# aspuru-guzik-group/waveflow

Hardware: AMD Instinct MI355X
Metric: flow log-prob evals/sec (higher is better)
Workload: dtype f32

## Files before the change

### waveflow_amd/build.py

```python
import os
import subprocess
import sys
from concurrent.futures import ThreadPoolExecutor

HERE = os.path.dirname(os.path.abspath(__file__))
CSRC = os.path.join(HERE, "csrc")
LIB = os.path.join(HERE, "libwaveflow_hip.so")
OBJ = os.path.join(CSRC, "_obj")

SOURCES = ["wf_tables.cpp", "wf_runtime.cpp", "wf_model_build.cpp", "wf_model_images.cpp", "wf_dispatch.cpp", "wf_train.cpp", "wf_kernels_scalar.hip", "wf_scalar_inst_d2.hip", "wf_scalar_inst_d3.hip", "wf_scalar_inst_d4.hip", "wf_scalar_inst_d56.hip",
           "wf_scalar_inst_d78.hip", "wf_scalar_inst_n64.hip", "wf_scalar_inst_n64_d56.hip",
           "wf_scalar_inst_n64_d78.hip", "wf_kernels_mfma.hip", "wf_mfma_inst_d2.hip", "wf_mfma_inst_d2t2.hip", "wf_mfma_inst_d34.hip",
           "wf_mfma_inst_d567.hip", "wf_mfma_inst_d8.hip", "wf_mfma_inst_k2.hip", "wf_kernels_rqs.hip", "wf_kernels_grad.hip", "wf_kernels_wave.hip", "wf_kernels_etile.hip",
           "wf_kernels_etile_bwd.hip", "wf_etile_bwd_k2.hip", "wf_kernels_etile_sample.hip", "wf_kernels_etile_dir.hip", "wf_kernels_spline.hip"]
FLAGS = ["--offload-arch=gfx950", "-O3", "-std=c++17", "-fPIC", "-ffp-contract=off", "-Wall", "-Wno-unused-function"]
FLAGS += ["-mllvm", "-amdgpu-prealloc-sgpr-spill-vgprs"]
FLAGS += os.environ.get("WF_CXXFLAGS", "").split()
MFMA_FLAGS = ["-fno-slp-vectorize", "-Xclang", "-target-feature", "-Xclang", "-packed-fp32-ops"]
EXTRA_FLAGS = {"wf_etile_bwd_k2.hip": ["-mllvm", "-amdgpu-sched-strategy=max-ilp"]}


def _hipcc():
    for c in (os.environ.get("HIPCC"), "/opt/rocm/bin/hipcc", "hipcc"):
        if c and (os.path.isabs(c) and os.path.exists(c) or not os.path.isabs(c)):
            return c
    return "hipcc"


def _deps(obj):
    try:
        text = open(obj + ".d").read()
    except OSError:
        return None
    words = text.replace("\\\n", " ").split()
    if len(words) < 2 or not words[0].endswith(":"):
        return None
    return words[1:]


def _stale(obj):
    deps = _deps(obj)
    try:
        t = os.path.getmtime(obj)
        return deps is None or any(os.path.getmtime(d) > t for d in deps)
    except OSError:
        return True


STAMP = os.path.join(HERE, "libwaveflow_hip.flags")


def _flags_text():
    return " ".join(FLAGS) + " | " + " ".join(MFMA_FLAGS) + " | " + " ".join(f"{k}: {' '.join(v)}" for k, v in sorted(EXTRA_FLAGS.items()))


def _library_current():
    try:
        if open(STAMP).read() != _flags_text():
            return False
        t = os.path.getmtime(LIB)
    except OSError:
        return False
    deps = [os.path.join(CSRC, f) for f in os.listdir(CSRC) if f.endswith((".hip", ".cpp", ".h"))]
    deps.append(os.path.join(HERE, "..", "include", "waveflow_hip.h"))
    return all(os.path.getmtime(d) <= t for d in deps if os.path.exists(d))


def build(force=False, verbose=False):
    if not force and _library_current():
        return LIB
    os.makedirs(OBJ, exist_ok=True)
    try:
        force = force or open(STAMP).read() != _flags_text()
    except OSError:
        force = True
    srcs = [s for s in SOURCES if os.path.exists(os.path.join(CSRC, s))]
    jobs = []
    for s in srcs:
        o = os.path.join(OBJ, s + ".o")
        if force or _stale(o):
            cmd = [_hipcc()] + FLAGS + (MFMA_FLAGS if ("mfma" in s or "etile" in s) else []) + EXTRA_FLAGS.get(s, []) + (["-x", "hip"] if s.endswith(".cpp") else [])
            cmd += ["-MD", "-MF", o + ".d", "-c", os.path.join(CSRC, s), "-o", o]
            jobs.append(cmd)

    def run(cmd):
        if verbose:
            print(" ".join(cmd), flush=True)
        r = subprocess.run(cmd, capture_output=True, text=True)
        if r.returncode != 0:
            raise RuntimeError("hipcc failed:\n" + " ".join(cmd) + "\n" + r.stdout + r.stderr)
        return r

    if jobs:
        with ThreadPoolExecutor(max_workers=min(os.cpu_count() or 4, 16, len(jobs))) as ex:
            list(ex.map(run, jobs))
    objs = [os.path.join(OBJ, s + ".o") for s in srcs]
    if jobs or force or not os.path.exists(LIB) or any(os.path.getmtime(LIB) < os.path.getmtime(o) for o in objs):
        tmp = LIB + ".tmp"
        run([_hipcc(), "--offload-arch=gfx950", "-shared", "-fPIC", "-o", tmp] + objs)
        if os.environ.get("WF_SKIP_ISA_GUARD") != "1":
            import importlib.util
            spec = importlib.util.spec_from_file_location("wf_isa_guard", os.path.join(HERE, "isa_guard.py"))
            isa_guard = importlib.util.module_from_spec(spec)
            spec.loader.exec_module(isa_guard)
            try:
                isa_guard.check(tmp)
            except Exception:
                os.remove(tmp)
                raise
        os.replace(tmp, LIB)
    with open(STAMP, "w") as f:
        f.write(_flags_text())
    return LIB


if __name__ == "__main__":
    print(build(force="--force" in sys.argv, verbose=True))
```

### waveflow_amd/csrc/wf_kernels_scalar.hip

```cpp
#include "wf_scalar_impl.h"

namespace wf {

namespace scalar {
WF_SCALAR_SHAPE(extern, 2, 32) WF_SCALAR_SHAPE(extern, 3, 32) WF_SCALAR_SHAPE(extern, 4, 32) WF_SCALAR_SHAPE(extern, 5, 32)
WF_SCALAR_SHAPE(extern, 6, 32) WF_SCALAR_SHAPE(extern, 7, 32) WF_SCALAR_SHAPE(extern, 8, 32)
WF_SCALAR_SHAPE(extern, 2, 64) WF_SCALAR_SHAPE(extern, 3, 64) WF_SCALAR_SHAPE(extern, 4, 64) WF_SCALAR_SHAPE(extern, 5, 64)
WF_SCALAR_SHAPE(extern, 6, 64) WF_SCALAR_SHAPE(extern, 7, 64) WF_SCALAR_SHAPE(extern, 8, 64)
}

namespace {
using namespace scalar;

constexpr int kSumBlock = 256;
constexpr int kSumMaxBlocks = 1024;

__device__ __forceinline__ void block_reduce2(double& a, double& b, double* sm) {
    sm[threadIdx.x] = a;
    sm[kSumBlock + threadIdx.x] = b;
    __syncthreads();
    for (int s = kSumBlock / 2; s > 0; s >>= 1) {
        if ((int)threadIdx.x < s) {
            sm[threadIdx.x] += sm[threadIdx.x + s];
            sm[kSumBlock + threadIdx.x] += sm[kSumBlock + threadIdx.x + s];
        }
        __syncthreads();
    }
    a = sm[0];
    b = sm[kSumBlock];
}

__device__ __forceinline__ void ring_push(double s, double q, double n, double* __restrict__ ring, int ring_len, unsigned long long* __restrict__ counter) {
    const unsigned long long c = *counter;
    double* slot = ring + (c % (unsigned long long)ring_len) * 3;
    slot[0] = s; slot[1] = q; slot[2] = n;
    *counter = c + 1;
}

__global__ __launch_bounds__(kSumBlock) void k_sums_stage1(const float* __restrict__ v, int64_t B, double* __restrict__ partial,
                                                           double* __restrict__ final, double* __restrict__ ring, int ring_len,
                                                           unsigned long long* __restrict__ counter) {
    __shared__ double sm[2 * kSumBlock];
    double s = 0.0, q = 0.0;
    for (int64_t i = (int64_t)blockIdx.x * kSumBlock + threadIdx.x; i < B; i += (int64_t)gridDim.x * kSumBlock) {
        const double x = (double)v[i];
        s += x;
        q += x * x;
    }
    block_reduce2(s, q, sm);
    if (threadIdx.x == 0) {
        if (final) {
            final[0] = s;
            final[1] = q;
            final[2] = (double)B;
            if (ring) ring_push(s, q, (double)B, ring, ring_len, counter);
        } else {
            partial[2 * blockIdx.x] = s;
            partial[2 * blockIdx.x + 1] = q;
        }
    }
}

__global__ __launch_bounds__(kSumBlock) void k_sums_stage2(const double* __restrict__ partial, int n_blocks, int64_t B, double* __restrict__ out,
                                                           double* __restrict__ ring, int ring_len, unsigned long long* __restrict__ counter) {
    __shared__ double sm[2 * kSumBlock];
    double s = 0.0, q = 0.0;
    for (int i = threadIdx.x; i < n_blocks; i += kSumBlock) {
        s += partial[2 * i];
        q += partial[2 * i + 1];
    }
    block_reduce2(s, q, sm);
    if (threadIdx.x == 0) {
        out[0] = s;
        out[1] = q;
        out[2] = (double)B;
        if (ring) ring_push(s, q, (double)B, ring, ring_len, counter);
    }
}

int sums_blocks(int64_t B) {
    int64_t n = (B + kSumBlock - 1) / kSumBlock;
    if (n < 1) n = 1;
    if (n > kSumMaxBlocks) n = kSumMaxBlocks;
    return (int)n;
}

int finish_launch() {
    hipError_t e = hipGetLastError();
    if (e != hipSuccess) {
        set_hip_error((int)e);
        return WF_ERR_HIP;
    }
    return WF_OK;
}

}

#define WF_DISPATCH_D(D_, NBP_, CALL)                                         \
    if ((NBP_) == 32) {                                                          \
        switch (D_) {                                                            \
            case 2: CALL(2, 32); break;                                          \
            case 3: CALL(3, 32); break;                                          \
            case 4: CALL(4, 32); break;                                          \
            case 5: CALL(5, 32); break;                                          \
            case 6: CALL(6, 32); break;                                          \
            case 7: CALL(7, 32); break;                                          \
            case 8: CALL(8, 32); break;                                          \
            default: return WF_ERR_UNSUPPORTED;                                  \
        }                                                                        \
    } else if ((NBP_) == 64) {                                                   \
        switch (D_) {                                                            \
            case 2: CALL(2, 64); break;                                          \
            case 3: CALL(3, 64); break;                                          \
            case 4: CALL(4, 64); break;                                          \
            case 5: CALL(5, 64); break;                                          \
            case 6: CALL(6, 64); break;                                          \
            case 7: CALL(7, 64); break;                                          \
            case 8: CALL(8, 64); break;                                          \
            default: return WF_ERR_UNSUPPORTED;                                  \
        }                                                                        \
    } else {                                                                     \
        return WF_ERR_UNSUPPORTED;                                               \
    }

int launch_scalar(const ModelDev& md, const ModelDev* md_dev, int mode, const float* x, int64_t B, float* out, float* u, int32_t* idx,
                  void* stream) {
    hipStream_t s = (hipStream_t)stream;
#define CALL(DD, NN) run_eval<DD, NN>(md_dev, mode, x, B, out, u, idx, s)
    WF_DISPATCH_D(md.D, md.nbp, CALL)
#undef CALL
    return finish_launch();
}

int launch_scalar_layer(const ModelDev& md, const ModelDev* md_dev, int layer, const float* u_in, int64_t B, float* y, float* logdet,
                        int32_t* idx, void* stream) {
    hipStream_t s = (hipStream_t)stream;
#define CALL(DD, NN) run_layer<DD, NN>(md_dev, layer, u_in, B, y, logdet, idx, s)
    WF_DISPATCH_D(md.D, md.nbp, CALL)
#undef CALL
    return finish_launch();
}

int launch_scalar_inverse(const ModelDev& md, const ModelDev* md_dev, const float* u, int64_t B, float* x, int exact, void* stream) {
    hipStream_t s = (hipStream_t)stream;
#define CALL(DD, NN) run_inverse<DD, NN>(md_dev, u, B, x, exact, s)
    WF_DISPATCH_D(md.D, md.nbp, CALL)
#undef CALL
    return finish_launch();
}

int launch_scalar_sample(const ModelDev& md, const ModelDev* md_dev, unsigned long long seed, int64_t B, float* x, float* latent, int exact,
                         void* stream) {
    hipStream_t s = (hipStream_t)stream;
#define CALL(DD, NN) run_sample<DD, NN>(md_dev, seed, B, x, latent, exact, s)
    WF_DISPATCH_D(md.D, md.nbp, CALL)
#undef CALL
    return finish_launch();
}

__global__ void k_sort_rows(const float* __restrict__ x, int64_t B, int D, float* __restrict__ xs, int32_t* __restrict__ inv) {
    const int64_t b = (int64_t)blockIdx.x * blockDim.x + threadIdx.x;
    if (b >= B) return;
    float r[WF_MAX_DIM];
    for (int d = 0; d < D; ++d) r[d] = x[b * D + d];
    int n = 0;
    for (int pass = 0; pass < D; ++pass)
        for (int i = pass & 1; i + 1 < D; i += 2)
            if (r[i] > r[i + 1]) {
                const float t = r[i]; r[i] = r[i + 1]; r[i + 1] = t;
                ++n;
            }
    if (xs)
        for (int d = 0; d < D; ++d) xs[b * D + d] = r[d];
    if (inv) inv[b] = n;
}
__global__ void k_apply_sign(float* __restrict__ v, const int32_t* __restrict__ inv, int64_t B) {
    const int64_t b = (int64_t)blockIdx.x * blockDim.x + threadIdx.x;
    if (b < B && (inv[b] & 1)) v[b] = -v[b];
}

int launch_sort_rows(const float* x, int64_t B, int D, float* xs, int32_t* inv, void* stream) {
    if (B <= 0) return WF_OK;
    hipLaunchKernelGGL(k_sort_rows, dim3((unsigned)((B + 255) / 256)), dim3(256), 0, (hipStream_t)stream, x, B, D, xs, inv);
    return finish_launch();
}
int launch_apply_sign(float* v, const int32_t* inv, int64_t B, void* stream) {
    if (B <= 0) return WF_OK;
    hipLaunchKernelGGL(k_apply_sign, dim3((unsigned)((B + 255) / 256)), dim3(256), 0, (hipStream_t)stream, v, inv, B);
    return finish_launch();
}

int64_t block_sums_ws_bytes(int64_t) { return (int64_t)kSumMaxBlocks * 2 * sizeof(double); }

int launch_block_sums(const float* v, int64_t B, double* out, void* ws, int64_t, void* stream, double* ring, int ring_len,
                      unsigned long long* counter) {
    hipStream_t s = (hipStream_t)stream;
    const int nb = sums_blocks(B);
    double* partial = (double*)ws;
    if (nb == 1) {
        hipLaunchKernelGGL(k_sums_stage1, dim3(1), dim3(kSumBlock), 0, s, v, B, partial, out, ring, ring_len, counter);
        return finish_launch();
    }
    hipLaunchKernelGGL(k_sums_stage1, dim3(nb), dim3(kSumBlock), 0, s, v, B, partial, (double*)nullptr, (double*)nullptr, 0,
                       (unsigned long long*)nullptr);
    hipLaunchKernelGGL(k_sums_stage2, dim3(1), dim3(kSumBlock), 0, s, (const double*)partial, nb, B, out, ring, ring_len, counter);
    return finish_launch();
}

}
```

### waveflow_amd/csrc/wf_mfma_impl.h

```cpp
#pragma once
#include <hip/hip_runtime.h>

#include <cstdlib>

#include "wf_internal.h"

#define WF_PIN() __builtin_amdgcn_sched_barrier(0)

namespace wf {
namespace mfma {

using f32x16 = __attribute__((ext_vector_type(16))) float;
using f32x4 = __attribute__((ext_vector_type(4))) float;
using i32x2 = __attribute__((ext_vector_type(2))) int;
using f32x2 = __attribute__((ext_vector_type(2))) float;
using f16x8 = __attribute__((ext_vector_type(8))) _Float16;

__device__ __forceinline__ float act_tanh(float xs) {
    return __builtin_fmaf(-2.0f, __builtin_amdgcn_rcpf(__builtin_amdgcn_exp2f(xs) + 1.0f), 1.0f);
}
__device__ __forceinline__ float act_sigmoid(float xs) {
    return __builtin_amdgcn_rcpf(1.0f + __builtin_amdgcn_exp2f(xs));
}
__device__ __forceinline__ float fast_log(float x) {
    return __builtin_amdgcn_logf(x) * 0.6931471805599453f;
}

__device__ __forceinline__ float xhalf_sum(float v) {
    const unsigned u = __float_as_uint(v);
    const auto s = __builtin_amdgcn_permlane32_swap(u, u, false, false);
    return __uint_as_float(s[0]) + __uint_as_float(s[1]);
}

__device__ __forceinline__ f32x4 load4(const float* p) { return *reinterpret_cast<const f32x4*>(p); }
__device__ __forceinline__ float uniform_f(float v) {
    float r;
    asm("v_readfirstlane_b32 %0, %1" : "=s"(r) : "v"(v));
    return r;
}
__device__ __forceinline__ float xhalf_max(float v) {
    const unsigned u = __float_as_uint(v);
    const auto s = __builtin_amdgcn_permlane32_swap(u, u, false, false);
    return fmaxf(__uint_as_float(s[0]), __uint_as_float(s[1]));
}

__device__ __forceinline__ f32x16 load16(const float* p) {
    const f32x4* q = reinterpret_cast<const f32x4*>(p);
    const f32x4 a = q[0], b = q[1], c = q[2], d = q[3];
    return f32x16{a[0], a[1], a[2], a[3], b[0], b[1], b[2], b[3], c[0], c[1], c[2], c[3], d[0], d[1], d[2], d[3]};
}

struct Lerp {
    int il, ir, xl, xr;
    float t;
};

__device__ __forceinline__ int wrap_clamp(int i, int n) {
    if (i < 0) i += n;
    return min(max(i, 0), n - 1);
}

__device__ __forceinline__ float div_by_n(float xl, float n, float rn, int exact_div) {
    if (exact_div) return xl / n;
    const float q = xl * rn;
    const float r = __builtin_fmaf(-q, n, xl);
    return __builtin_fmaf(r, rn, q);
}

__device__ __forceinline__ Lerp make_lerp(float x, int n_mesh, float rn, int exact_div) {
    Lerp L;
    const int n_points = n_mesh - 1;
    const float xs = x * (float)n_points;
    const float fl = floorf(xs);
    L.xl = (int)fl;
    L.xr = (int)ceilf(xs);
    L.il = wrap_clamp(L.xl, n_mesh);
    L.ir = wrap_clamp(L.xr, n_mesh);
    const float dx = x - div_by_n(fl, (float)n_points, rn, exact_div);
    L.t = L.il == L.ir ? 0.0f : dx * (float)n_points;
    return L;
}

__device__ __forceinline__ bool any_far(const Lerp& Lp);
__device__ __forceinline__ f32x2 comp_lerp(const f32x4* __restrict__ comp2, const Lerp& Lp) {
    const f32x4 c = comp2[Lp.il];
    float b0 = c[2], b1 = c[3];
    if (any_far(Lp)) {
        const f32x4 r = comp2[Lp.ir];
        const bool far = Lp.ir != Lp.il && Lp.ir != Lp.il + 1;
        b0 = far ? r[0] : b0;
        b1 = far ? r[1] : b1;
    }
    return f32x2{__builtin_fmaf(b0 - c[0], Lp.t, c[0]), __builtin_fmaf(b1 - c[1], Lp.t, c[1])};
}

struct Frag {
    f16x8 hi[2], lo[2];
};
using u32x4 = __attribute__((ext_vector_type(4))) unsigned;
using f16x2 = __attribute__((ext_vector_type(2))) _Float16;
__device__ __forceinline__ void split8(const float (&r)[8], f16x8& hi, f16x8& lo) {
    u32x4 H, L;
    asm volatile(
        "s_nop 0\n\t"
        "v_cvt_pk_f16_f32 %0, %8, %9\n\tv_cvt_pk_f16_f32 %1, %10, %11\n\tv_cvt_pk_f16_f32 %2, %12, %13\n\tv_cvt_pk_f16_f32 %3, %14, %15\n\t"
        "v_fma_mixhi_f16 %4, %0, -1.0, %9 op_sel:[1,0,0] op_sel_hi:[1,0,0]\n\t"
        "v_fma_mixhi_f16 %5, %1, -1.0, %11 op_sel:[1,0,0] op_sel_hi:[1,0,0]\n\t"
        "v_fma_mixhi_f16 %6, %2, -1.0, %13 op_sel:[1,0,0] op_sel_hi:[1,0,0]\n\t"
        "v_fma_mixhi_f16 %7, %3, -1.0, %15 op_sel:[1,0,0] op_sel_hi:[1,0,0]\n\t"
        "v_fma_mixlo_f16 %4, %0, -1.0, %8 op_sel_hi:[1,0,0]\n\t"
        "v_fma_mixlo_f16 %5, %1, -1.0, %10 op_sel_hi:[1,0,0]\n\t"
        "v_fma_mixlo_f16 %6, %2, -1.0, %12 op_sel_hi:[1,0,0]\n\t"
        "v_fma_mixlo_f16 %7, %3, -1.0, %14 op_sel_hi:[1,0,0]\n\t"
        "s_nop 1"
        : "=&v"(H[0]), "=&v"(H[1]), "=&v"(H[2]), "=&v"(H[3]), "=&v"(L[0]), "=&v"(L[1]), "=&v"(L[2]), "=&v"(L[3])
        : "v"(r[0]), "v"(r[1]), "v"(r[2]), "v"(r[3]), "v"(r[4]), "v"(r[5]), "v"(r[6]), "v"(r[7]));
    hi = __builtin_bit_cast(f16x8, H);
    lo = __builtin_bit_cast(f16x8, L);
}
template <int T>
__device__ __forceinline__ void mfma_step(const _Float16* Wh, const _Float16* Wl, int kt, int s, const Frag (&in)[T][2], f32x16 (&acc)[T], int lane) {
    const f16x8 ah = *reinterpret_cast<const f16x8*>(Wh + ((kt * 2 + s) * 64 + lane) * 8);
    const f16x8 al = *reinterpret_cast<const f16x8*>(Wl + ((kt * 2 + s) * 64 + lane) * 8);
#pragma unroll
    for (int t = 0; t < T; ++t) acc[t] = __builtin_amdgcn_mfma_f32_32x32x16_f16(al, in[t][kt].hi[s], acc[t], 0, 0, 0);
#pragma unroll
    for (int t = 0; t < T; ++t) acc[t] = __builtin_amdgcn_mfma_f32_32x32x16_f16(ah, in[t][kt].lo[s], acc[t], 0, 0, 0);
#pragma unroll
    for (int t = 0; t < T; ++t) acc[t] = __builtin_amdgcn_mfma_f32_32x32x16_f16(ah, in[t][kt].hi[s], acc[t], 0, 0, 0);
}
template <int T>
__device__ __forceinline__ void dense64_block(const _Float16* Wh, const _Float16* Wl, const Frag (&in)[T][2], f32x16 (&acc)[T], int lane) {
#pragma unroll
    for (int kt = 0; kt < 2; ++kt)
#pragma unroll
        for (int s = 0; s < 2; ++s) mfma_step<T>(Wh, Wl, kt, s, in, acc, lane);
}
template <int T>
__device__ __forceinline__ void act8(const f32x16 (&x)[T], int s, Frag (&f)[T][2], int ob) {
#pragma unroll
    for (int t = 0; t < T; ++t) {
        float r[8];
#pragma unroll
        for (int j = 0; j < 8; ++j) r[j] = __builtin_amdgcn_rcpf(__builtin_amdgcn_exp2f(x[t][8 * s + j]) + 1.0f);
        split8(r, f[t][ob].hi[s], f[t][ob].lo[s]);
    }
}

template <int D, int NBK>
struct NetOff {
    static constexpr int S0 = (D + 1) / 2;
    static constexpr int W0 = 0;
    static constexpr int b0 = W0 + 2 * S0 * 64;
    static constexpr int W1h = b0 + 64;
    static constexpr int W1l = W1h + 2048;
    static constexpr int b1 = W1l + 2048;
    static constexpr int W2h = b1 + 64;
    static constexpr int W2l = W2h + (D - 1) * NBK * 1024;
// ... 90 lines not shown
    WF_PIN();
    mfma_step<T>(W2h, W2l, 1, 0, h2, o, lane);
    mfma_step<T>(W2h, W2l, 1, 1, h2, o, lane);
}

__device__ __forceinline__ int med3i(int x, int lo, int hi) {
    int r;
    asm("v_med3_i32 %0, %1, %2, %3" : "=v"(r) : "v"(x), "v"(lo), "v"(hi));
    return r;
}
template <int NBK, int NO, bool FAR>
__device__ __forceinline__ void fetch_block(f32x16 (&A)[NO], f32x16 (&Bv)[NO], const float* __restrict__ tab, const Lerp& Lp, int h, const float* bnd, int kb) {
    const char* tb = reinterpret_cast<const char*>(tab);
    constexpr unsigned kRec = 32u * NO, kMesh = 8u * NBK * kRec;
    const bool far = FAR && Lp.ir != Lp.il && Lp.ir != Lp.il + 1;
#pragma unroll
    for (int q = 0; q < 4; ++q) {
        const i32x2 lh = *reinterpret_cast<const i32x2*>(bnd + (kb * 2 + h) * 16 + q * 2);
        const unsigned off = (unsigned)med3i(Lp.il, lh[0], lh[1]) * kMesh + (unsigned)(8 * kb + 2 * q + h) * kRec;
        unsigned offb = off + 16u;
        if (FAR) {
            const unsigned offr = (unsigned)med3i(Lp.ir, lh[0], lh[1]) * kMesh + (unsigned)(8 * kb + 2 * q + h) * kRec;
            offb = far ? offr : offb;
        }
#pragma unroll
        for (int o = 0; o < NO; ++o) {
            const f32x4 a = load4(reinterpret_cast<const float*>(tb + off + o * 32)), b = load4(reinterpret_cast<const float*>(tb + offb + o * 32));
#pragma unroll
            for (int e = 0; e < 4; ++e) { A[o][q * 4 + e] = a[e]; Bv[o][q * 4 + e] = b[e]; }
        }
    }
}
template <int NO>
__device__ __forceinline__ void block_dot(const f32x16& v, const f32x16 (&A)[NO], const f32x16 (&Bv)[NO], float t, float (&part)[NO]) {
    float sa[NO][2], sb[NO][2];
#pragma unroll
    for (int o = 0; o < NO; ++o) sa[o][0] = sa[o][1] = sb[o][0] = sb[o][1] = 0.0f;
#pragma unroll
    for (int r = 0; r < 16; r += 2)
#pragma unroll
        for (int o = 0; o < NO; ++o) {
            sa[o][0] = __builtin_fmaf(v[r], A[o][r], sa[o][0]);
            sb[o][0] = __builtin_fmaf(v[r], Bv[o][r], sb[o][0]);
            sa[o][1] = __builtin_fmaf(v[r + 1], A[o][r + 1], sa[o][1]);
            sb[o][1] = __builtin_fmaf(v[r + 1], Bv[o][r + 1], sb[o][1]);
        }
#pragma unroll
    for (int o = 0; o < NO; ++o) {
        const float Aa = sa[o][0] + sa[o][1], Bb = sb[o][0] + sb[o][1];
        part[o] += __builtin_fmaf(Bb - Aa, t, Aa);
    }
}
template <int NBK, int NO, bool FAR>
__device__ __forceinline__ void rows_lerp_dot(const f32x16 (&v)[NBK], const float* __restrict__ tab, const Lerp& Lp, int h, const float* bnd, float (&out)[NO],
                                              const float* __restrict__ rsum = nullptr, float* rl = nullptr, float* rr = nullptr) {
    auto row_sums = [&]() {
        if (rsum) {
            static_assert(NO <= 2, "row sums: orders 0 and 1");
            const f32x4 c = load4(rsum + (size_t)Lp.il * 4);
            f32x4 r = c;
            bool far = false;
            if (FAR) {
                far = Lp.ir != Lp.il && Lp.ir != Lp.il + 1;
                r = load4(rsum + (size_t)Lp.ir * 4);
            }
#pragma unroll
            for (int o = 0; o < NO; ++o) {
                rl[o] = c[o];
                rr[o] = far ? r[o] : c[2 + o];
            }
        }
    };
    float part[NO];
#pragma unroll
    for (int o = 0; o < NO; ++o) part[o] = 0.0f;
    if (NBK > 1) row_sums();
#pragma unroll
    for (int kb = 0; kb < NBK; ++kb) {
        f32x16 A[NO], Bv[NO];
        if (kb > 0) __builtin_amdgcn_sched_barrier(0);
        fetch_block<NBK, NO, FAR>(A, Bv, tab, Lp, h, bnd, kb);
        if (NBK == 1) row_sums();
        block_dot<NO>(v[kb], A, Bv, Lp.t, part);
    }
#pragma unroll
    for (int o = 0; o < NO; ++o) out[o] = xhalf_sum(part[o]);
}
__device__ __forceinline__ bool any_far(const Lerp& Lp) { return __builtin_amdgcn_ballot_w64(Lp.ir != Lp.il && Lp.ir != Lp.il + 1) != 0; }

template <int NBK>
__device__ __forceinline__ float rows_dot(const f32x16 (&v)[NBK], const float* __restrict__ tab, const Lerp& Lp, int h, const float* bnd) {
    float out[1];
    if (!any_far(Lp)) rows_lerp_dot<NBK, 1, false>(v, tab, Lp, h, bnd, out);
    else rows_lerp_dot<NBK, 1, true>(v, tab, Lp, h, bnd, out);
    return out[0];
}

template <int NBK>
__device__ __forceinline__ void ispline_eval(const f32x16 (&v)[NBK], const float* __restrict__ tab, const float* __restrict__ rsum, const Lerp& Lp, int h,
                                             const float* bnd, float rS, float rs, float& y, float& logdy) {
    float num[2], rl[2], rr[2];
    if (!any_far(Lp)) rows_lerp_dot<NBK, 2, false>(v, tab, Lp, h, bnd, num, rsum, rl, rr);
    else rows_lerp_dot<NBK, 2, true>(v, tab, Lp, h, bnd, num, rsum, rl, rr);
    const float ynum = __builtin_fmaf(rs, __builtin_fmaf(rr[0] - rl[0], Lp.t, rl[0]), num[0]);
    const float dnum = __builtin_fmaf(rs, __builtin_fmaf(rr[1] - rl[1], Lp.t, rl[1]), num[1]);
    y = ynum * rS;
    logdy = fast_log(__builtin_fmaf(dnum, rS, 1e-7f));
}

template <int NBK>
__device__ __forceinline__ void sigmoid_block(f32x16 (&o)[NBK], const float* fk_lds , int h, float& S1, float& Sf,
                                              bool gate = false, float g = 1.0f, const float* z_lds = nullptr) {
    float s1 = 0.0f, sf = 0.0f;
#pragma unroll
    for (int kb = 0; kb < NBK; ++kb) {
        const f32x16 fk = load16(fk_lds + (kb * 2 + h) * 16);
        f32x16 zz = fk;
        if (gate) zz = load16(z_lds + (kb * 2 + h) * 16);
#pragma unroll
        for (int r = 0; r < 16; ++r) {
            float v = act_sigmoid(o[kb][r]);
            if (gate) v = __builtin_fmaf(g, v, zz[r]);
            o[kb][r] = v;
            s1 += v;
            sf = __builtin_fmaf(v, fk[r], sf);
        }
    }
    S1 = xhalf_sum(s1);
    Sf = xhalf_sum(sf);
}

template <int kThreads>
__device__ __forceinline__ void stage_floats(const float* __restrict__ src, float* dst, int n_floats) {
    const f32x4* s4 = reinterpret_cast<const f32x4*>(src);
    f32x4* d4 = reinterpret_cast<f32x4*>(dst);
    const int n4 = n_floats >> 2;
    for (int base = threadIdx.x; base < n4; base += kThreads * 8) {
        f32x4 v[8];
#pragma unroll
        for (int u = 0; u < 8; ++u) {
            const int i = base + u * kThreads;
            if (i < n4) v[u] = s4[i];
        }
#pragma unroll
        for (int u = 0; u < 8; ++u) {
            const int i = base + u * kThreads;
            if (i < n4) d4[i] = v[u];
        }
    }
}

template <int D, int NBK, int kWaves, int T, bool IDX, bool SPEC>
__global__ __launch_bounds__(kWaves * 64) void k_mfma(const MfmaDev mm, int mode_in, const float* __restrict__ xg, int64_t B,
                                                      float* __restrict__ out, float* __restrict__ u_out, int32_t* __restrict__ idx_out) {
    const int mode = mode_in & 3;
    const bool presort = (mode_in & 4) != 0;
    extern __shared__ __attribute__((aligned(16))) float lds[];
    constexpr int kThreads = kWaves * 64;
    const int box_kind = SPEC ? (int)WF_BOX_MEAN : mm.box_kind, layer_kind = SPEC ? (int)WF_LAYER_IMADE : mm.layer_kind;
    const int prior_kind = SPEC ? (int)WF_PRIOR_WAVEFLOW : mm.prior_kind, staged = (SPEC && D == 2) ? 0 : mm.staged, exact_div = SPEC ? 0 : mm.exact_div;
    __shared__ int next_slot;
    if (threadIdx.x == 0) next_slot = 0;
    stage_floats<kThreads>(mm.image + mm.const_img_off, lds, mm.const_floats);
    if (!staged) stage_floats<kThreads>(mm.image, lds + mm.const_floats, mm.net_floats * mm.n_nets);
    __syncthreads();

    const int lane = threadIdx.x & 63, wave = threadIdx.x >> 6;
    const int j = lane & 31, h = lane >> 5;
    const float* fkI = lds;
    const float* fkP = lds + 32 * NBK;
    const float* ob2b = lds + 64 * NBK;
    const float* bndI = ob2b + NBK * NBK * 1024;
    const float* bndP = bndI + 32 * NBK;
    const float* cbP = bndP + 32 * NBK;
    float* slots = lds + mm.const_floats;
    const int64_t n_tiles = (B + 31) >> 5;
    constexpr int kTilesPerChunk = kWaves * T;
    const int64_t n_chunks = (n_tiles + kTilesPerChunk - 1) / kTilesPerChunk;
    const int idx_stride = (mm.n_layers + 1) * D * 2;
    const float L = mm.box_L, tol = 1e-7f;
    const float rn_mesh = 1.0f / (float)(mm.n_mesh - 1);
    const float box_space0 = uniform_f(2 * L + tol), box_nlog0 = uniform_f(0.0f - fast_log(2 * L + tol));
    int f16_bad = 0;
    if (mm.f16_ovf)
        for (int n = 0; n < mm.n_nets; ++n) f16_bad |= mm.f16_ovf[n];
    const int64_t my_chunks = n_chunks > (int64_t)blockIdx.x ? (n_chunks - blockIdx.x + gridDim.x - 1) / gridDim.x : 0;
    const int my_slots = (int)(my_chunks * kWaves);
    auto tile_ids = [&](int64_t chunk, int wpos, int64_t (&w)[T], bool (&valid)[T], int32_t* (&idx)[T]) __attribute__((always_inline)) {
#pragma unroll
        for (int t = 0; t < T; ++t) {
            const int64_t tile = (chunk * kWaves + wpos) * T + t;
            w[t] = tile * 32 + j;
            valid[t] = w[t] < B;
            idx[t] = (IDX && idx_out && valid[t] && h == 0) ? idx_out + w[t] * idx_stride : nullptr;
        }
    };
    auto load_box = [&](const int64_t (&w)[T], const bool (&valid)[T], float (&cur)[T][D], float (&logdet)[T]) __attribute__((always_inline)) {
        float nxt[T][D];
#pragma unroll
        for (int t = 0; t < T; ++t) {
            const int64_t wl = valid[t] ? w[t] : B - 1;
#pragma unroll
            for (int d = 0; d < D; ++d) cur[t][d] = xg[wl * D + d];
            if (presort) {
#pragma unroll
                for (int r = 0; r < D; ++r)
#pragma unroll
                    for (int i = r & 1; i + 1 < D; i += 2) {
                        const float a = cur[t][i], b = cur[t][i + 1];
                        const bool sw = a > b;
                        cur[t][i] = sw ? b : a;
                        cur[t][i + 1] = sw ? a : b;
                    }
            }
        }
#pragma unroll
        for (int t = 0; t < T; ++t) {
            float ld = 0.0f;
            if (box_kind == WF_BOX_MEAN) {
                float s = 0.0f;
#pragma unroll
                for (int d = 0; d < D; ++d) s = s + cur[t][d];
                const float mean = s / (float)D;
                const float l = mean - cur[t][0];
                const float wd = cur[t][D - 1] - cur[t][0];
                float space_left = 2 * L;
#pragma unroll
                for (int i = 0; i < D - 1; ++i) {
                    const float diff = cur[t][i + 1] - cur[t][i];
                    nxt[t][i] = diff / (i == 0 ? box_space0 : space_left + tol);
                    ld = i == 0 ? box_nlog0 : ld - fast_log(space_left + tol);
                    space_left = space_left - diff;
                }
                nxt[t][D - 1] = (mean + L - l) / (2 * L - wd + tol);
                ld = ld - fast_log(2 * L - wd + tol);
#pragma unroll
                for (int d = 0; d < D; ++d) cur[t][d] = nxt[t][d];
            } else if (box_kind == WF_BOX_FIRST) {
                nxt[t][0] = (cur[t][0] + L) / (2 * L);
                float ls = 0.0f;
#pragma unroll
                for (int i = 1; i < D; ++i) nxt[t][i] = (cur[t][i] - cur[t][i - 1]) / (L - cur[t][i - 1] + tol);
#pragma unroll
                for (int i = 0; i < D - 1; ++i) ls = ls + fast_log(L - cur[t][i] + tol);
                ld = -fast_log(2 * L) - ls;
#pragma unroll
                for (int d = 0; d < D; ++d) cur[t][d] = nxt[t][d];
            }
            logdet[t] = ld;
        }

    };
    auto flow_layer = [&](int l, const float* net, float (&cur)[T][D], float (&logdet)[T], int32_t* (&idx)[T]) __attribute__((always_inline)) {
        float nxt[T][D];
        {
            Frag h2[T][2];
            f32x16 pend[T];
            hidden_layers<D, NBK, T>(net, cur, lane, h2, pend);
            if (layer_kind == WF_LAYER_IMADE) {
#pragma unroll
                for (int t = 0; t < T; ++t) {
                    const Lerp Lp = make_lerp(cur[t][0], mm.n_mesh, rn_mesh, exact_div);
                    if (IDX && idx[t]) { idx[t][(l * D) * 2] = Lp.xl; idx[t][(l * D) * 2 + 1] = Lp.xr; }
                    const f32x2 c0 = comp_lerp(mm.comp2 + (size_t)l * mm.n_mesh, Lp);
                    nxt[t][0] = c0[0];
                    logdet[t] = logdet[t] + fast_log(c0[1] + 1e-7f);
                }
                const bool gate_i = !SPEC && mm.i_gate != 0;
                float gl[T];
#pragma unroll
                for (int t = 0; t < T; ++t) gl[t] = 1.0f;
#pragma unroll (D)
                for (int d = 1; d < D; ++d) {
                    if (D > 4) __builtin_amdgcn_sched_barrier(0);
                    if (gate_i) {
#pragma unroll
                        for (int t = 0; t < T; ++t) gl[t] = gl[t] * (cur[t][d - 1] * cur[t][d - 1] * cur[t][d - 1]);
                    }
                    f32x16 v[T][NBK];
#pragma unroll
                    for (int kb = 0; kb < NBK; ++kb) {
                        f32x16 o[T];
                        if (d == 1 && kb == 0) out_block_first<D, NBK, T>(net, h2, pend, lane, o);
                        else out_block<D, NBK, T>(net, h2, d, kb, lane, o);
#pragma unroll
                        for (int t = 0; t < T; ++t) v[t][kb] = o[t];
                    }
#pragma unroll
                    for (int t = 0; t < T; ++t) {
                        float S1, Sf;
                        sigmoid_block<NBK>(v[t], fkI, h, S1, Sf, gate_i, gl[t], net + NetOff<D, NBK>::z + d * NBK * 32);
                        const float rs = mm.i_reg * S1;
                        const float rS = __builtin_amdgcn_rcpf(__builtin_fmaf(rs, mm.F_I, Sf));
                        const Lerp Lp = make_lerp(cur[t][d], mm.n_mesh, rn_mesh, exact_div);
                        if (IDX && idx[t]) { idx[t][(l * D + d) * 2] = Lp.xl; idx[t][(l * D + d) * 2 + 1] = Lp.xr; }
                        float ld;
                        ispline_eval<NBK>(v[t], mm.tabI, mm.rsI, Lp, h, bndI, rS, rs, nxt[t][d], ld);
                        logdet[t] = logdet[t] + ld;
                    }
                }
            } else {
                float ls[T];
#pragma unroll
                for (int t = 0; t < T; ++t) ls[t] = 0.0f;
#pragma unroll
                for (int d = 0; d < D; ++d) {
                    if (d == 0) {
// ... 69 lines not shown
                            if (d == 1 && kb == 0) out_block_first<D, NBK, T>(net, h2, pend, lane, o[kb]);
                            else out_block<D, NBK, T>(net, h2, d, kb, lane, o[kb]);
                        }
#pragma unroll
                        for (int t = 0; t < T; ++t) {
                            float s1 = 0.0f, amax = 0.0f;
                            if (gate_p) {
#pragma unroll
                                for (int kb = 0; kb < NBK; ++kb) {
                                    const f32x16 zz = load16(net + NetOff<D, NBK>::z + (d * NBK + kb) * 32 + h * 16);
#pragma unroll
                                    for (int r = 0; r < 16; ++r) o[kb][t][r] = __builtin_fmaf(gp[t], o[kb][t][r], zz[r]);
                                }
                            }
#pragma unroll
                            for (int kb = 0; kb < NBK; ++kb) {
                                const f32x16 keep = load16(fkP + (kb * 2 + h) * 16);
#pragma unroll
                                for (int r = 0; r < 16; ++r) {
                                    s1 += o[kb][t][r];
                                    o[kb][t][r] = o[kb][t][r] * keep[r];
                                    amax = fmaxf(amax, fabsf(o[kb][t][r]));
                                }
                            }
                            s1 = xhalf_sum(s1);
                            amax = xhalf_max(amax);
                            const int ex = amax > 0.0f ? __builtin_amdgcn_frexp_expf(amax) : 0;
                            const float scale = mm.prior_quotient ? 1.0f / s1 : __builtin_amdgcn_ldexpf(1.0f, -ex);
                            Frag of[NBK];
#pragma unroll
                            for (int kb = 0; kb < NBK; ++kb)
#pragma unroll
                                for (int s = 0; s < 2; ++s) {
                                    float r8[8];
#pragma unroll
                                    for (int jj = 0; jj < 8; ++jj) r8[jj] = o[kb][t][8 * s + jj] * scale;
                                    split8(r8, of[kb].hi[s], of[kb].lo[s]);
                                }
                            f32x16 c[NBK];
                            float n2 = 0.0f;
                            const _Float16* obh = reinterpret_cast<const _Float16*>(ob2b);
#pragma unroll
                            for (int ko = 0; ko < NBK; ++ko) {
                                c[ko] = f32x16{0, 0, 0, 0, 0, 0, 0, 0, 0, 0, 0, 0, 0, 0, 0, 0};
#pragma unroll
                                for (int ki = 0; ki < NBK; ++ki)
#pragma unroll
                                    for (int s = 0; s < 2; ++s) {
                                        const _Float16* blk = obh + (size_t)(ko * NBK + ki) * 2048;
                                        const f16x8 ah = *reinterpret_cast<const f16x8*>(blk + (s * 64 + lane) * 8);
                                        const f16x8 al = *reinterpret_cast<const f16x8*>(blk + 1024 + (s * 64 + lane) * 8);
                                        c[ko] = __builtin_amdgcn_mfma_f32_32x32x16_f16(al, of[ki].hi[s], c[ko], 0, 0, 0);
                                        c[ko] = __builtin_amdgcn_mfma_f32_32x32x16_f16(ah, of[ki].lo[s], c[ko], 0, 0, 0);
                                        c[ko] = __builtin_amdgcn_mfma_f32_32x32x16_f16(ah, of[ki].hi[s], c[ko], 0, 0, 0);
                                    }
                                if (!SPEC && mm.p_bias) {
                                    const float bs = scale * s1;
                                    const f32x16 cb = load16(cbP + (ko * 2 + h) * 16);
#pragma unroll
                                    for (int r = 0; r < 16; ++r) c[ko][r] = __builtin_fmaf(bs, cb[r], c[ko][r]);
                                }
#pragma unroll
                                for (int r = 0; r < 16; ++r) n2 = __builtin_fmaf(c[ko][r], c[ko][r], n2);
                            }
                            const float rnorm = __builtin_amdgcn_rsqf(xhalf_sum(n2));
                            const float v0 = rows_dot<NBK>(c, mm.tabP, Lp[t], h, bndP) * rnorm;
                            val[t] = (s1 < 0.0f && !mm.prior_quotient) ? -v0 : v0;
                        }
                    } else {
                        f32x16 v[T][NBK];
#pragma unroll
                        for (int kb = 0; kb < NBK; ++kb) {
                            f32x16 o[T];
                            if (d == 1 && kb == 0) out_block_first<D, NBK, T>(net, h2, pend, lane, o);
                            else out_block<D, NBK, T>(net, h2, d, kb, lane, o);
#pragma unroll
                            for (int t = 0; t < T; ++t) v[t][kb] = o[t];
                        }
#pragma unroll
                        for (int t = 0; t < T; ++t) {
                            float S1, Sf;
                            sigmoid_block<NBK>(v[t], fkP, h, S1, Sf, gate_p, gp[t], net + NetOff<D, NBK>::z + d * NBK * 32);
                            val[t] = rows_dot<NBK>(v[t], mm.tabP, Lp[t], h, bndP) * __builtin_amdgcn_rcpf(Sf);
                        }
                    }
#pragma unroll
                    for (int t = 0; t < T; ++t) {
                        if (wavefn) {
                            const bool constrained = (mm.constrained_mask >> d) & 1u;
                            if (mode == 0) {
                                float pr = val[t] * val[t];
                                if (constrained) pr = pr * 0.5f;
                                lp[t] = lp[t] + fast_log(pr + 1e-7f);
                            } else {
                                const float vv = constrained ? val[t] * 0.70710678118654752f : val[t];
                                prod[t] = prod[t] * vv;
                            }
                        } else {
                            lp[t] = lp[t] + fast_log(val[t] + 1e-7f);
                        }
                        nxt[t][d] = uc[t];
                    }
                }
#pragma unroll
                for (int t = 0; t < T; ++t) {
                    result[t] = (wavefn && mode != 0) ? prod[t] * __expf(0.5f * logdet[t]) : lp[t] + logdet[t];
#pragma unroll
                    for (int d = 0; d < D; ++d) cur[t][d] = nxt[t][d];
                }
            } else if (prior_kind == WF_PRIOR_UNIFORM) {
#pragma unroll
                for (int t = 0; t < T; ++t) {
#pragma unroll
                    for (int d = 0; d < D; ++d) cur[t][d] = fminf(fmaxf(cur[t][d], 0.0f), 1.0f);
                    result[t] = logdet[t];
                }
            } else {
#pragma unroll
                for (int t = 0; t < T; ++t) {
                    float lpn = 0.0f;
#pragma unroll
                    for (int d = 0; d < D; ++d) {
                        const float z = cur[t][d] + mm.normal_offset;
                        lpn = lpn + (1.8378770664093453f + z * z) * -0.5f;
                    }
                    result[t] = lpn + logdet[t];
                }
            }
        }
#pragma unroll
        for (int t = 0; t < T; ++t)
            if (valid[t] && h == 0) {
                if (f16_bad) result[t] = __builtin_nanf("");
                if (presort && mode == 1) {
                    int inv = 0;
                    float xr[D];
#pragma unroll
                    for (int d = 0; d < D; ++d) xr[d] = xg[w[t] * D + d];
#pragma unroll
                    for (int i = 0; i < D; ++i)
#pragma unroll
                        for (int k = i + 1; k < D; ++k) inv += xr[i] > xr[k] ? 1 : 0;
                    if (inv & 1) result[t] = -result[t];
                }
                out[w[t]] = result[t];
                if (u_out) {
#pragma unroll
                    for (int d = 0; d < D; ++d) u_out[w[t] * D + d] = cur[t][d];
                }
            }
    };

    if (!staged) {
        for (;;) {
            int q = 0;
            if (lane == 0) q = __hip_atomic_fetch_add(&next_slot, 1, __ATOMIC_RELAXED, __HIP_MEMORY_SCOPE_WORKGROUP);
            q = __builtin_amdgcn_readfirstlane(q);
            if (q >= my_slots) break;
            const int64_t chunk = (int64_t)blockIdx.x + (int64_t)(q / kWaves) * gridDim.x;
            float cur[T][D], logdet[T];
            int64_t w[T];
            bool valid[T];
            int32_t* idx[T];
            tile_ids(chunk, q % kWaves, w, valid, idx);
            load_box(w, valid, cur, logdet);
            for (int l = 0; l < mm.n_layers; ++l) flow_layer(l, slots + (size_t)l * mm.net_floats, cur, logdet, idx);
            head_store(slots + (size_t)mm.n_layers * mm.net_floats, cur, logdet, w, valid, idx);
        }
    } else {
        float* state = slots + mm.net_floats + (size_t)wave * kStagedGroups * T * (D + 1) * 32;
        const int tps = mm.staged_groups;
        const int64_t n_super = (n_chunks + tps - 1) / tps;
        const bool prior_net = mode != 2 && (prior_kind == WF_PRIOR_WAVEFLOW || prior_kind == WF_PRIOR_MFLOW);
        for (int64_t sc = blockIdx.x; sc < n_super; sc += gridDim.x) {
            for (int p = 0; p <= mm.n_layers; ++p) {
                if (p < mm.n_layers || prior_net) {
                    __syncthreads();
                    stage_floats<kThreads>(mm.image + (size_t)p * mm.net_floats, slots, mm.net_floats);
                    __syncthreads();
                }
                for (int g = 0; g < tps; ++g) {
                    const int64_t chunk = sc * tps + g;
                    if (chunk >= n_chunks) break;
                    float cur[T][D], logdet[T];
                    int64_t w[T];
                    bool valid[T];
                    int32_t* idx[T];
                    tile_ids(chunk, wave, w, valid, idx);
                    float* st = state + (size_t)g * T * (D + 1) * 32;
                    if (p == 0) load_box(w, valid, cur, logdet);
                    else {
#pragma unroll
                        for (int t = 0; t < T; ++t) {
#pragma unroll
                            for (int d = 0; d < D; ++d) cur[t][d] = st[(t * (D + 1) + d) * 32 + j];
                            logdet[t] = st[(t * (D + 1) + D) * 32 + j];
                        }
                    }
                    if (p < mm.n_layers) {
                        flow_layer(p, slots, cur, logdet, idx);
                        if (h == 0) {
#pragma unroll
                            for (int t = 0; t < T; ++t) {
#pragma unroll
                                for (int d = 0; d < D; ++d) st[(t * (D + 1) + d) * 32 + j] = cur[t][d];
                                st[(t * (D + 1) + D) * 32 + j] = logdet[t];
                            }
                        }
                    } else head_store(slots, cur, logdet, w, valid, idx);
                }
            }
        }
    }
}

template <int D, int NBK, int kWaves, int T, bool IDX, bool SPEC>
int launch_dwi(const MfmaDev* mdev, int lds_bytes, int mode, const float* x, int64_t B, float* out, float* u, int32_t* idx, hipStream_t s) {
    static DynLdsSlots cfg{};
    if (int rc = ensure_dynamic_lds(reinterpret_cast<const void*>(k_mfma<D, NBK, kWaves, T, IDX, SPEC>), lds_bytes, &cfg)) return rc;
    const int64_t n_tiles = (B + 31) / 32;
    const int64_t n_chunks = (n_tiles + kWaves * T - 1) / (kWaves * T);
    MfmaDev md = *mdev;
    int64_t grid = n_chunks;
    if (md.staged) {
        int64_t g = (n_chunks + 255) / 256;
        md.staged_groups = (int)(g < 1 ? 1 : (g > kStagedGroups ? kStagedGroups : g));
        grid = (n_chunks + md.staged_groups - 1) / md.staged_groups;
    }
    if (grid > 256) grid = 256;
    hipLaunchKernelGGL((k_mfma<D, NBK, kWaves, T, IDX, SPEC>), dim3((unsigned)grid), dim3(kWaves * 64), lds_bytes, s, md, mode, x, B, out, u, idx);
    hipError_t e = hipGetLastError();
    if (e != hipSuccess) {
        set_hip_error((int)e);
        return WF_ERR_HIP;
    }
    return WF_OK;
}

template <int D, int NBK, int kWaves, int T>
int launch_dw(const MfmaDev* mdev, int lds_bytes, int mode, const float* x, int64_t B, float* out, float* u, int32_t* idx, hipStream_t s) {
    if (idx) {
        if constexpr (T == 1) return launch_dwi<D, NBK, kWaves, 1, true, false>(mdev, lds_bytes, mode, x, B, out, u, idx, s);
        else return WF_ERR_UNSUPPORTED;
    }
    if constexpr (D == 2 || (D == 8 && NBK == 1)) {
        if (mdev->box_kind == WF_BOX_MEAN && mdev->layer_kind == WF_LAYER_IMADE && mdev->prior_kind == WF_PRIOR_WAVEFLOW && (D > 2 || !mdev->staged) &&
            !mdev->exact_div && !mdev->i_gate && !mdev->p_gate && !mdev->p_bias)
            return launch_dwi<D, NBK, kWaves, T, false, true>(mdev, lds_bytes, mode, x, B, out, u, nullptr, s);
    }
    return launch_dwi<D, NBK, kWaves, T, false, false>(mdev, lds_bytes, mode, x, B, out, u, nullptr, s);
}

}
}
```

Before: 4.183 billion.

## Add per-stream device tickets for fused sum reduction and D=2 tail work pool

Adds a per-device pool of atomic ticket words handed out per stream or per graph capture. The sums reduction now runs as one kernel in which the last block to finish does the final combine, replacing the separate stage-2 launch. The D=2 non-staged MFMA kernel splits its work into a statically owned part and a final round of chunks that all blocks claim dynamically through a global atomic, to even out tail imbalance. It adds a hipStreamIsCapturing query, a mutex and map lookup per launch, and relies on the ticket being reset correctly between launches on the same stream.

```diff
diff --git a/waveflow_amd/build.py b/waveflow_amd/build.py
--- a/waveflow_amd/build.py
+++ b/waveflow_amd/build.py
@@ -8,7 +8,7 @@
 LIB = os.path.join(HERE, "libwaveflow_hip.so")
 OBJ = os.path.join(CSRC, "_obj")
 
-SOURCES = ["wf_tables.cpp", "wf_runtime.cpp", "wf_model_build.cpp", "wf_model_images.cpp", "wf_dispatch.cpp", "wf_train.cpp", "wf_kernels_scalar.hip", "wf_scalar_inst_d2.hip", "wf_scalar_inst_d3.hip", "wf_scalar_inst_d4.hip", "wf_scalar_inst_d56.hip",
+SOURCES = ["wf_tables.cpp", "wf_runtime.cpp", "wf_model_build.cpp", "wf_model_images.cpp", "wf_dispatch.cpp", "wf_train.cpp", "wf_tickets.cpp", "wf_kernels_scalar.hip", "wf_scalar_inst_d2.hip", "wf_scalar_inst_d3.hip", "wf_scalar_inst_d4.hip", "wf_scalar_inst_d56.hip",
            "wf_scalar_inst_d78.hip", "wf_scalar_inst_n64.hip", "wf_scalar_inst_n64_d56.hip",
            "wf_scalar_inst_n64_d78.hip", "wf_kernels_mfma.hip", "wf_mfma_inst_d2.hip", "wf_mfma_inst_d2t2.hip", "wf_mfma_inst_d34.hip",
            "wf_mfma_inst_d567.hip", "wf_mfma_inst_d8.hip", "wf_mfma_inst_k2.hip", "wf_kernels_rqs.hip", "wf_kernels_grad.hip", "wf_kernels_wave.hip", "wf_kernels_etile.hip",
diff --git a/waveflow_amd/csrc/wf_kernels_scalar.hip b/waveflow_amd/csrc/wf_kernels_scalar.hip
--- a/waveflow_amd/csrc/wf_kernels_scalar.hip
+++ b/waveflow_amd/csrc/wf_kernels_scalar.hip
@@ -1,4 +1,5 @@
 #include "wf_scalar_impl.h"
+#include "wf_tickets.h"
 
 namespace wf {
 
@@ -68,6 +69,46 @@
     for (int i = threadIdx.x; i < n_blocks; i += kSumBlock) {
         s += partial[2 * i];
         q += partial[2 * i + 1];
+    }
+    block_reduce2(s, q, sm);
+    if (threadIdx.x == 0) {
+        out[0] = s;
+        out[1] = q;
+        out[2] = (double)B;
+        if (ring) ring_push(s, q, (double)B, ring, ring_len, counter);
+    }
+}
+
+__global__ __launch_bounds__(kSumBlock) void k_sums_fused(const float* __restrict__ v, int64_t B, double* partial, double* __restrict__ out,
+                                                          double* __restrict__ ring, int ring_len, unsigned long long* __restrict__ counter,
+                                                          unsigned long long* ticket) {
+    __shared__ double sm[2 * kSumBlock + 1];
+    double s = 0.0, q = 0.0;
+    for (int64_t i = (int64_t)blockIdx.x * kSumBlock + threadIdx.x; i < B; i += (int64_t)gridDim.x * kSumBlock) {
+        const double x = (double)v[i];
+        s += x;
+        q += x * x;
+    }
+    block_reduce2(s, q, sm);
+    if (threadIdx.x == 0) {
+        __hip_atomic_store(&partial[2 * blockIdx.x], s, __ATOMIC_RELAXED, __HIP_MEMORY_SCOPE_AGENT);
+        __hip_atomic_store(&partial[2 * blockIdx.x + 1], q, __ATOMIC_RELAXED, __HIP_MEMORY_SCOPE_AGENT);
+        __threadfence();
+        const unsigned long long t = __hip_atomic_fetch_add(ticket, 1ull, __ATOMIC_RELAXED, __HIP_MEMORY_SCOPE_AGENT);
+        const bool last = t == (unsigned long long)gridDim.x - 1;
+        if (last) {
+            __hip_atomic_store(ticket, 0ull, __ATOMIC_RELAXED, __HIP_MEMORY_SCOPE_AGENT);
+            __threadfence();
+        }
+        sm[2 * kSumBlock] = last ? 1.0 : 0.0;
+    }
+    __syncthreads();
+    if (sm[2 * kSumBlock] == 0.0) return;
+    const int n_blocks = (int)gridDim.x;
+    s = 0.0; q = 0.0;
+    for (int i = threadIdx.x; i < n_blocks; i += kSumBlock) {
+        s += __hip_atomic_load(&partial[2 * i], __ATOMIC_RELAXED, __HIP_MEMORY_SCOPE_AGENT);
+        q += __hip_atomic_load(&partial[2 * i + 1], __ATOMIC_RELAXED, __HIP_MEMORY_SCOPE_AGENT);
     }
     block_reduce2(s, q, sm);
     if (threadIdx.x == 0) {
@@ -201,6 +242,10 @@
         hipLaunchKernelGGL(k_sums_stage1, dim3(1), dim3(kSumBlock), 0, s, v, B, partial, out, ring, ring_len, counter);
         return finish_launch();
     }
+    if (unsigned long long* ticket = ticket_for_launch(stream)) {
+        hipLaunchKernelGGL(k_sums_fused, dim3(nb), dim3(kSumBlock), 0, s, v, B, partial, out, ring, ring_len, counter, ticket);
+        return finish_launch();
+    }
     hipLaunchKernelGGL(k_sums_stage1, dim3(nb), dim3(kSumBlock), 0, s, v, B, partial, (double*)nullptr, (double*)nullptr, 0,
                        (unsigned long long*)nullptr);
     hipLaunchKernelGGL(k_sums_stage2, dim3(1), dim3(kSumBlock), 0, s, (const double*)partial, nb, B, out, ring, ring_len, counter);
diff --git a/waveflow_amd/csrc/wf_mfma_impl.h b/waveflow_amd/csrc/wf_mfma_impl.h
--- a/waveflow_amd/csrc/wf_mfma_impl.h
+++ b/waveflow_amd/csrc/wf_mfma_impl.h
@@ -4,6 +4,7 @@
 #include <cstdlib>
 
 #include "wf_internal.h"
+#include "wf_tickets.h"
 
 #define WF_PIN() __builtin_amdgcn_sched_barrier(0)
 
@@ -400,7 +401,8 @@
 
 template <int D, int NBK, int kWaves, int T, bool IDX, bool SPEC>
 __global__ __launch_bounds__(kWaves * 64) void k_mfma(const MfmaDev mm, int mode_in, const float* __restrict__ xg, int64_t B,
-                                                      float* __restrict__ out, float* __restrict__ u_out, int32_t* __restrict__ idx_out) {
+                                                      float* __restrict__ out, float* __restrict__ u_out, int32_t* __restrict__ idx_out,
+                                                      unsigned long long* ticket) {
     const int mode = mode_in & 3;
     const bool presort = (mode_in & 4) != 0;
     extern __shared__ __attribute__((aligned(16))) float lds[];
@@ -776,20 +778,45 @@
     };
 
     if (!staged) {
+        constexpr bool kPool = D == 2 && !IDX;
+        int own_slots = my_slots, pool_slots = 0;
+        int64_t pool_first = n_chunks;
+        if constexpr (kPool) {
+            if (ticket) {
+                pool_first = n_chunks > (int64_t)gridDim.x ? n_chunks - gridDim.x : 0;
+                own_slots = pool_first > (int64_t)blockIdx.x ? (int)((pool_first - blockIdx.x + gridDim.x - 1) / gridDim.x) * kWaves : 0;
+                pool_slots = (int)(n_chunks - pool_first) * kWaves;
+            }
+        }
         for (;;) {
             int q = 0;
             if (lane == 0) q = __hip_atomic_fetch_add(&next_slot, 1, __ATOMIC_RELAXED, __HIP_MEMORY_SCOPE_WORKGROUP);
             q = __builtin_amdgcn_readfirstlane(q);
-            if (q >= my_slots) break;
-            const int64_t chunk = (int64_t)blockIdx.x + (int64_t)(q / kWaves) * gridDim.x;
+            int64_t chunk = (int64_t)blockIdx.x + (int64_t)(q / kWaves) * gridDim.x;
+            int wpos = q % kWaves;
+            if (q >= own_slots) {
+                if (!kPool || pool_slots == 0) break;
+                unsigned p = 0;
+                if (lane == 0) p = (unsigned)__hip_atomic_fetch_add(ticket, 1ull, __ATOMIC_RELAXED, __HIP_MEMORY_SCOPE_AGENT);
+                p = (unsigned)__builtin_amdgcn_readfirstlane((int)p);
+                if (p >= (unsigned)pool_slots) break;
+                chunk = pool_first + (int64_t)(p / kWaves);
+                wpos = (int)(p % kWaves);
+            }
             float cur[T][D], logdet[T];
             int64_t w[T];
             bool valid[T];
             int32_t* idx[T];
-            tile_ids(chunk, q % kWaves, w, valid, idx);
+            tile_ids(chunk, wpos, w, valid, idx);
             load_box(w, valid, cur, logdet);
             for (int l = 0; l < mm.n_layers; ++l) flow_layer(l, slots + (size_t)l * mm.net_floats, cur, logdet, idx);
             head_store(slots + (size_t)mm.n_layers * mm.net_floats, cur, logdet, w, valid, idx);
+        }
+        if constexpr (kPool) {
+            if (ticket && lane == 0) {
+                const unsigned long long left = __hip_atomic_fetch_add(ticket, 1ull << 32, __ATOMIC_RELAXED, __HIP_MEMORY_SCOPE_AGENT);
+                if ((unsigned)(left >> 32) == gridDim.x * kWaves - 1) __hip_atomic_store(ticket, 0ull, __ATOMIC_RELAXED, __HIP_MEMORY_SCOPE_AGENT);
+            }
         }
     } else {
         float* state = slots + mm.net_floats + (size_t)wave * kStagedGroups * T * (D + 1) * 32;
@@ -852,7 +879,10 @@
         grid = (n_chunks + md.staged_groups - 1) / md.staged_groups;
     }
     if (grid > 256) grid = 256;
-    hipLaunchKernelGGL((k_mfma<D, NBK, kWaves, T, IDX, SPEC>), dim3((unsigned)grid), dim3(kWaves * 64), lds_bytes, s, md, mode, x, B, out, u, idx);
+    unsigned long long* ticket = nullptr;
+    if constexpr (D == 2 && !IDX)
+        if (!md.staged) ticket = ticket_for_launch(s);
+    hipLaunchKernelGGL((k_mfma<D, NBK, kWaves, T, IDX, SPEC>), dim3((unsigned)grid), dim3(kWaves * 64), lds_bytes, s, md, mode, x, B, out, u, idx, ticket);
     hipError_t e = hipGetLastError();
     if (e != hipSuccess) {
         set_hip_error((int)e);
diff --git a/waveflow_amd/csrc/wf_tickets.cpp b/waveflow_amd/csrc/wf_tickets.cpp
--- /dev/null
+++ b/waveflow_amd/csrc/wf_tickets.cpp
@@ -0,0 +1,58 @@
+#include "wf_tickets.h"
+
+#include <hip/hip_runtime.h>
+
+#include <mutex>
+
+#include "wf_internal.h"
+
+namespace wf {
+
+namespace {
+
+struct DevicePool {
+    unsigned long long* words = nullptr;
+    TicketBook* book = nullptr;
+};
+std::mutex g_mutex;
+DevicePool g_pools[kMaxDevices];
+
+bool create_pool(DevicePool& p) {
+    void* q = nullptr;
+    if (hipMalloc(&q, (size_t)kTicketWords * sizeof(unsigned long long)) != hipSuccess) {
+        (void)hipGetLastError();
+        return false;
+    }
+    if (hipMemset(q, 0, (size_t)kTicketWords * sizeof(unsigned long long)) != hipSuccess || hipStreamSynchronize(nullptr) != hipSuccess) {
+        (void)hipGetLastError();
+        (void)hipFree(q);
+        (void)hipGetLastError();
+        return false;
+    }
+    p.words = (unsigned long long*)q;
+    p.book = new TicketBook(kTicketWords);
+    return true;
+}
+
+}
+
+unsigned long long* ticket_for_launch(void* stream) {
+    int dev = 0;
+    if (hipGetDevice(&dev) != hipSuccess || dev < 0 || dev >= kMaxDevices) {
+        (void)hipGetLastError();
+        return nullptr;
+    }
+    hipStreamCaptureStatus st = hipStreamCaptureStatusNone;
+    if (hipStreamIsCapturing((hipStream_t)stream, &st) != hipSuccess) {
+        (void)hipGetLastError();
+        return nullptr;
+    }
+    const bool capturing = st != hipStreamCaptureStatusNone;
+    std::lock_guard<std::mutex> lock(g_mutex);
+    DevicePool& p = g_pools[dev];
+    if (!p.words && (capturing || !create_pool(p))) return nullptr;
+    const int w = capturing ? p.book->capture_word() : p.book->stream_word(stream);
+    return w >= 0 ? p.words + w : nullptr;
+}
+
+}
diff --git a/waveflow_amd/csrc/wf_tickets.h b/waveflow_amd/csrc/wf_tickets.h
--- /dev/null
+++ b/waveflow_amd/csrc/wf_tickets.h
@@ -0,0 +1,31 @@
+#pragma once
+
+#include <cstdint>
+#include <unordered_map>
+
+namespace wf {
+
+constexpr int kTicketWords = 4096;
+
+class TicketBook {
+public:
+    explicit TicketBook(int n_words) : n_words_(n_words > 0 ? n_words : 0) {}
+    int stream_word(const void* stream) {
+        auto it = by_stream_.find(stream);
+        if (it != by_stream_.end()) return it->second;
+        if (next_ >= n_words_) return -1;
+        by_stream_.emplace(stream, next_);
+        return next_++;
+    }
+    int capture_word() { return next_ < n_words_ ? next_++ : -1; }
+    int words_left() const { return n_words_ - next_; }
+    int size() const { return n_words_; }
+
+private:
+    int n_words_, next_ = 0;
+    std::unordered_map<const void*, int> by_stream_;
+};
+
+unsigned long long* ticket_for_launch(void* stream);
+
+}
```

Result: slower. 2.884 billion (-31.0%).
